# the3cloud/zktls

Hardware: AMD Instinct MI355X
Metric: trace-cells/s (higher is better)
Workload: dtype u32

## Files before the change

### zktls_amd/csrc/kernels.h

```cpp
#pragma once
#include <hip/hip_runtime.h>
#include <stddef.h>
#include <stdint.h>

#include "babybear.cuh"

namespace zk {

struct NttPassArgs {
    const uint32_t* in;
    uint32_t* out;
    uint64_t in_ld, out_ld;
    uint32_t ncols;
    uint32_t num_tiles;
    uint32_t log_m;
    uint64_t in_tile_mul, in_stride;
    uint64_t out_tile_mul, out_stride;
    uint32_t bitrev_out;
    uint32_t map_mode;
    uint64_t tile_perm;
    uint32_t fast_path;
    uint32_t debug_flags;
    uint32_t cols_per_thread;
    uint32_t bench_tag;
// ... 169 lines not shown
    uint32_t inv_zh[4];
    const uint32_t* body;
    uint32_t n_constraints;
    const uint32_t* weights;
    const uint32_t* pub;
    uint32_t* out;
    uint32_t* lde_out; uint64_t lde_ld;
    const uint32_t* recs; uint32_t n_terms; uint32_t n_public;
    const uint32_t* addend;
    uint32_t no_chain;
    uint32_t wide;
    uint32_t cls[6];
};
constexpr uint32_t AIR_WIDE_POINTS = 64, AIR_WIDE_PITCH = 65;
inline bool air_wide_form(uint32_t width, uint32_t n_terms, int log_n, uint32_t n_public) {
    return n_terms >= 2048 && width % 4 == 0 && (size_t)AIR_WIDE_PITCH * (width + AIR_SLOT_EXTRA + n_public) * 4 <= 160 * 1024 && log_n >= 6;
}
ZK_HD uint32_t air_wide_word(uint32_t slot, uint32_t W) {
    if (slot < W) return AIR_WIDE_PITCH * slot;
    if (slot < 2 * W) return AIR_WIDE_PITCH * (slot - W) + 1u;
    return AIR_WIDE_PITCH * (W + (slot - 2 * W));
}
hipError_t launch_quotient_air(const QuotientAirArgs& a, hipStream_t s);

hipError_t launch_inv_denominators(const uint32_t* xs, uint64_t count, const Ext& z0, const Ext& z1, int npoints,
                                   uint32_t* out, uint32_t* xw, uint64_t xw_count, hipStream_t s);

struct OpenArgs {
    const uint32_t* mat;
    uint64_t ld;
    uint32_t width;
    uint64_t rows;
    const uint32_t* xw;
    uint64_t xw_stride;
    uint32_t* partial;
    int tx;
};
size_t open_chunks(uint64_t rows, uint32_t width, uint64_t ld, const uint32_t* mat);
hipError_t launch_open(const OpenArgs& a, int npts, const Ext& scale0, const Ext& scale1, uint32_t* out, hipStream_t s);

struct ReducedArgs {
    const uint32_t* tlde; uint64_t t_ld; uint32_t width;
    const uint32_t* qlde; uint64_t q_ld; uint32_t q_width;
    const uint32_t* plde; uint64_t p_ld; uint32_t p_width;
    uint64_t rows;
    const uint32_t* alpha_pow;
    const uint32_t* dinv;
    Ext y_loc, y_next, y_pl, y_pn, y_q, off_next, off_pl, off_pn, off_q;
    Ext off_loc;
    int accumulate;
    uint32_t* out;
};
hipError_t launch_reduced_opening(const ReducedArgs& a, uint32_t* scratch_at, hipStream_t s);

struct PermArgs {
    const uint32_t* trace; uint64_t ld;
    uint64_t rows; uint32_t pairs;
    Ext gamma, beta;
    uint32_t* out; uint64_t out_ld;
};
hipError_t launch_perm_trace(const PermArgs& a, uint32_t* block_scratch, hipStream_t s);

constexpr int LOOKUP_REC_WORDS = 12;
struct LookupArgs {
    const uint32_t* table; uint32_t ni, cols;
    Ext gamma, bpow[9];
    const uint8_t* cmap; uint32_t n_used, chunk_mask;
};
constexpr uint32_t LOOKUP_MAX_COLS = 512, LOOKUP_STAGE_MAX_USED = 56;
struct MachinePermArgs {
    LookupArgs lk;
    const uint32_t* trace; uint64_t ld; uint64_t rows;
    uint32_t* out; uint64_t out_ld;
    const uint32_t* pre; uint64_t pre_ld; uint32_t pre_w;
};
bool lookup_perm_two_sources_ok(const MachinePermArgs& a);
hipError_t launch_perm_trace_machine(const MachinePermArgs& a, uint32_t* block_scratch, hipStream_t s);
struct MachineQuotArgs {
    LookupArgs lk;
    const uint32_t* lde; uint64_t ld; const uint32_t* perm; uint64_t perm_ld; int log_n;
    int log_qd;
    const uint32_t* xs; const uint32_t* sel_first; const uint32_t* sel_last; uint32_t wn_inv;
    const uint32_t* weights;
    Ext cumsum;
    uint32_t* addend;
};
hipError_t launch_lookup_addend(const MachineQuotArgs& a, hipStream_t s);

hipError_t launch_fri_fold(const uint32_t* in, uint32_t* out, const uint32_t* itw, uint64_t half, const Ext& beta, hipStream_t s);
hipError_t launch_ext_add(uint32_t* dst, const uint32_t* src, uint64_t count, hipStream_t s);
hipError_t launch_fri_fold_dev(const uint32_t* in, uint32_t* out, const uint32_t* itw, uint64_t half, const uint32_t* beta_ptr,
                               int squarings, hipStream_t s);

struct DevChallenger {
    uint32_t state[16];
    uint32_t in[8];
    uint32_t out[8];
    int32_t n_in, n_out;
};
hipError_t launch_fri_challenge(DevChallenger* chal, const uint32_t* root, uint32_t* beta_out, uint32_t* root_log, hipStream_t s);


struct GrindArgs {
    uint32_t state[16];
    int slot;
    uint32_t mask;
// ... 15 lines not shown
```

### zktls_amd/csrc/prover.cpp

```cpp
#include <atomic>
#include <chrono>
#include <condition_variable>
#include <deque>
#include <cstring>
#include <functional>
#include <mutex>
#include <string>
#include <thread>
#include <vector>

#include "proof_common.h"
#include "batch.h"

namespace zk { std::atomic<bool> g_fri_graph{true}; }
namespace zk {

extern std::atomic<uint64_t> g_p2_generation;
void air_digest_cached(const AirView& a, uint32_t out[8]) {
    struct Entry { std::vector<uint32_t> words; uint64_t generation; uint32_t dg[8]; };
    static std::mutex mu;
    static std::vector<Entry> cache;
    const uint64_t gen = g_p2_generation.load();
    {
        std::lock_guard<std::mutex> lk(mu);
// ... 429 lines not shown
int zkhip_fri_fold_k(zkhip_ctx* ctx, const uint32_t* d_in, int log_h, int log_arity, const uint32_t beta[4], uint32_t* d_out) {
    CHECK_CTX(ctx);
    if (!d_in || !d_out || !beta || log_arity < 1 || log_arity > 6 || log_h < log_arity || log_h > MAX_LOG_ROWS + 3)
        return fail(ZKHIP_ERR_INVALID, "fri_fold_k: bad arguments");
    ZK_TRY(ensure_fold_table(ctx, log_h));
    void* tmp;
    ZK_TRY(ctx_reserve(ctx, S_PARTIAL, ((size_t)1 << log_h) * 16, &tmp));
    uint32_t* ping = (uint32_t*)tmp;
    uint32_t* pong = ping + ((size_t)2 << log_h);
    Ext b{{beta[0], beta[1], beta[2], beta[3]}};
    const uint32_t* src = d_in;
    for (int j = 0; j < log_arity; j++) {
        const int lh = log_h - j;
        uint32_t* dst = (j == log_arity - 1) ? d_out : ((j & 1) ? pong : ping);
        ZK_HIP(launch_fri_fold(src, dst, ctx->dom_itw, (uint64_t)1 << (lh - 1), b, ctx->stream));
        src = dst;
        b = ext_mul(b, b);
    }
    return ZKHIP_OK;
}

int zkhip_request_digest(const uint8_t* input, size_t input_len, const uint8_t* program, size_t program_len, uint32_t out[8]) {
    if (!out || (input_len && !input) || (program_len && !program)) return fail(ZKHIP_ERR_INVALID, "request_digest: null pointer");
    uint32_t st[16] = {0};
    int pos = 0;
    auto absorb = [&](uint32_t canonical) {
        st[pos++] = to_monty(canonical);
        if (pos == 8) { p2_permute(st); pos = 0; }
    };
    auto absorb_bytes = [&](const uint8_t* b, size_t n) {
        absorb((uint32_t)(n & 0xFFFFFF));
        absorb((uint32_t)((uint64_t)n >> 24) & 0xFFFFFF);
        for (size_t i = 0; i < n; i += 3) {
            uint32_t v = b[i];
            if (i + 1 < n) v |= (uint32_t)b[i + 1] << 8;
            if (i + 2 < n) v |= (uint32_t)b[i + 2] << 16;
            absorb(v);
        }
    };
    absorb(0x5A4B54);
    absorb_bytes(input, input_len);
    absorb_bytes(program, program_len);
    if (pos) p2_permute(st);
    for (int i = 0; i < 8; i++) out[i] = from_monty(st[i]);
    return ZKHIP_OK;
}

size_t zkhip_proof_size(int log_n, uint32_t width, const zkhip_params* prm, size_t n_public) {
    (void)n_public;
    if (check_shape(log_n, width, prm) != ZKHIP_OK) return 0;
    return proof_words(log_n, width, prm) * 4;
}

static int prove_shard_impl(zkhip_ctx* ctx, const uint32_t* d_trace, size_t ld, int log_n, uint32_t width,
                            const uint32_t* public_values, size_t n_public, const zkhip_params* prm,
                            uint8_t* proof, size_t cap, size_t* len, const AirView* air) {
    CHECK_CTX(ctx);
    ZK_TRY(check_shape(log_n, width, prm));
    if (!d_trace || !proof || !len || ld < width || (n_public && !public_values)) return fail(ZKHIP_ERR_INVALID, "prove_shard: bad arguments");
    for (size_t i = 0; i < n_public; i++) if (public_values[i] >= P) return fail(ZKHIP_ERR_INVALID, "prove_shard: public values must be canonical");
    if (air && prm->logup_pairs) return fail(ZKHIP_ERR_INVALID, "prove_shard_air: a constraint program excludes the built-in lookup argument (logup_pairs must be 0)");
    if (air && prm->code_width) return fail(ZKHIP_ERR_INVALID, "prove_shard_air: the code / data group split belongs to the built-in prover (code_width must be 0)");
    const int lqd = air ? air->lqd : 1;
    if (lqd > prm->log_blowup) return fail(ZKHIP_ERR_INVALID, "prove_shard_air: constraints of degree 4 or 5 need log_blowup >= 2 (the quotient domain must lie inside the committed LDE domain)");
    const size_t NQ = (size_t)1 << lqd, QW = 4 * NQ;
    const size_t need = proof_words(log_n, width, prm, air != nullptr, lqd) * 4;
    if (cap < need) return fail(ZKHIP_ERR_BUFFER, "prove_shard: proof buffer too small (see zkhip_proof_size)");
    *len = 0;
    Shape sh;
    shape_of(log_n, prm, sh);
    const int H = log_n + sh.b, Hq = log_n + lqd, Q = prm->num_queries;
    const int RL = sh.R, K = sh.K;
    const size_t n = (size_t)1 << log_n, m = (size_t)1 << H, arity = (size_t)1 << K;
    hipStream_t st = ctx->stream;
    ZK_TRY(ensure_domain(ctx, log_n, sh.b));

    uint32_t* pf = (uint32_t*)proof;
    size_t pos = 0;
    const uint32_t LQ = (uint32_t)prm->logup_pairs;
    const size_t wp = LQ ? 4 * ((size_t)LQ + 1) : 0;
    const uint32_t CW = sh.cw;
    pf[pos++] = PROOF_MAGIC; pf[pos++] = air ? 7u : (CW ? 8u : (sh.ext ? 3u : (LQ ? 2u : PROOF_VERSION))); pf[pos++] = (uint32_t)log_n; pf[pos++] = width;
    pf[pos++] = (uint32_t)prm->log_blowup; pf[pos++] = (uint32_t)Q; pf[pos++] = (uint32_t)prm->pow_bits; pf[pos++] = (uint32_t)n_public;
    if (sh.ext || air) { pf[pos++] = LQ; pf[pos++] = (uint32_t)sh.K; pf[pos++] = (uint32_t)sh.F; pf[pos++] = (uint32_t)sh.hw; }
    else if (LQ) pf[pos++] = LQ;
    if (air) { air_digest_cached(*air, pf + pos); pos += 8; }
    if (CW) pf[pos++] = CW;

    Challenger ch;
    transcript_init(ch, log_n, width, prm, n_public, sh, air);
    uint32_t root[8];

    void *v_tlde, *v_ttree;
    ZK_TRY(ctx_reserve(ctx, S_TLDE, m * width * 4, &v_tlde));
    ZK_TRY(ctx_reserve(ctx, S_TTREE, (2 * m - 1) * 32, &v_ttree));
    uint32_t* tlde = (uint32_t*)v_tlde; uint32_t* ttree = (uint32_t*)v_ttree;
    ZK_TRY(op_coset_lde(ctx, d_trace, ld, tlde, width, log_n, width, sh.b, MONTY_GEN));
    uint32_t* ctree = nullptr;
    if (CW) {
        void* v_ctree;
        ZK_TRY(ctx_reserve(ctx, S_CTREE, (2 * m - 1) * 32, &v_ctree));
        ctree = (uint32_t*)v_ctree;
        ZK_TRY(commit_hw(ctx, tlde, width, CW, H, ctree, sh.hw));
        ZK_TRY(d2h(ctx, root, ctree + (2 * m - 2) * 8, 32));
        for (int i = 0; i < 8; i++) { ch.observe(root[i]); pf[pos++] = from_monty(root[i]); }
        ZK_TRY(commit_hw(ctx, tlde + CW, width, width - CW, H, ttree, sh.hw));
// ... 53 lines not shown
    uint32_t* dinv = (uint32_t*)v_dinv; uint32_t* d_open = (uint32_t*)v_open;
    uint32_t* xw = dinv + 8 * m;
    ZK_HIP(launch_inv_denominators(ctx->dom_xs, m, zpts[0], zpts[1], 2, dinv, xw, n, st));
    ZK_TRY(run_open(ctx, tlde, width, log_n, width, zpts, 2, xw, d_open));
    ZK_TRY(dev_sync(ctx));
    if (LQ) {
        ZK_TRY(run_open(ctx, plde, wp, log_n, (uint32_t)wp, zpts, 2, xw, d_open + 8 * (size_t)width));
        ZK_TRY(dev_sync(ctx));
    }
    ZK_TRY(run_open(ctx, qlde, QW, log_n, (uint32_t)QW, zpts, 1, xw, d_open + 8 * (size_t)width + 8 * wp));
    std::vector<uint32_t> opened((2 * (size_t)width + 2 * wp + QW) * 4);
    ZK_TRY(d2h(ctx, opened.data(), d_open, opened.size() * 4));
    observe_words(ch, opened.data(), opened.size());
    for (size_t i = 0; i < opened.size(); i++) pf[pos++] = from_monty(opened[i]);
    const Ext* op_loc = (const Ext*)opened.data();
    const Ext* op_nxt = op_loc + width;
    const Ext* op_pl = op_nxt + width;
    const Ext* op_pn = op_pl + wp;
    const Ext* op_q = op_pn + wp;

    const Ext fa = ch.sample_ext();
    size_t np = width > QW ? width : QW;
    if (wp > np) np = wp;
    std::vector<Ext> fapow(np);
    fapow[0] = ext_one();
    for (size_t j = 1; j < np; j++) fapow[j] = ext_mul(fapow[j - 1], fa);
    ReducedArgs ra{};
    ra.y_loc = ra.y_next = ra.y_pl = ra.y_pn = ra.y_q = ext_zero();
    ra.off_loc = ext_one(); ra.accumulate = 0;
    for (size_t j = 0; j < width; j++) {
        ra.y_loc = ext_add(ra.y_loc, ext_mul(fapow[j], op_loc[j]));
        ra.y_next = ext_add(ra.y_next, ext_mul(fapow[j], op_nxt[j]));
    }
    for (size_t j = 0; j < wp; j++) {
        ra.y_pl = ext_add(ra.y_pl, ext_mul(fapow[j], op_pl[j]));
        ra.y_pn = ext_add(ra.y_pn, ext_mul(fapow[j], op_pn[j]));
    }
    for (size_t j = 0; j < QW; j++) ra.y_q = ext_add(ra.y_q, ext_mul(fapow[j], op_q[j]));
    ra.off_next = ext_pow(fa, width);
    ra.off_pl = ext_pow(fa, 2 * (uint64_t)width);
    ra.off_pn = ext_pow(fa, 2 * (uint64_t)width + wp);
    ra.off_q = ext_pow(fa, 2 * (uint64_t)width + 2 * wp);
    void *v_apf, *v_layers, *v_ltrees;
    ZK_TRY(ctx_reserve(ctx, S_APOW_F, np * 16, &v_apf));
    ZK_TRY(h2d(ctx, v_apf, fapow.data(), np * 16));
    ZK_TRY(ctx_reserve(ctx, S_FRI_LAYERS, 2 * m * 16, &v_layers));
    ZK_TRY(ctx_reserve(ctx, S_FRI_TREES, 2 * m * 32, &v_ltrees));
    uint32_t* layers = (uint32_t*)v_layers; uint32_t* ltrees = (uint32_t*)v_ltrees;
    ra.tlde = tlde; ra.t_ld = width; ra.width = width; ra.qlde = qlde; ra.q_ld = QW; ra.q_width = (uint32_t)QW; ra.rows = m;
    ra.plde = plde; ra.p_ld = wp; ra.p_width = (uint32_t)wp;
    ra.alpha_pow = (const uint32_t*)v_apf; ra.dinv = dinv; ra.out = layers;
    void* v_at;
    ZK_TRY(ctx_reserve(ctx, S_PARTIAL, 2 * m * 16, &v_at));
    ZK_HIP(launch_reduced_opening(ra, (uint32_t*)v_at, st));

    std::vector<size_t> layer_off(RL + 1), tree_off(RL + 1);
    {
        size_t lo = 0, to = 0;
        for (int l = 0; l <= RL; l++) {
            layer_off[l] = lo; tree_off[l] = to;
            lo += ((size_t)1 << (H - K * l)) * 4;
            if (l < RL) to += (2 * ((size_t)1 << (H - K * (l + 1))) - 1) * 8;
        }
    }
    ZK_TRY(fri_commit_phase(ctx, ch, sh, H, RL, layers, ltrees, layer_off, tree_off, (uint32_t*)v_at, m, nullptr, pf, pos));
    {
        const int lf = sh.F + sh.b;
        const size_t nf = (size_t)1 << lf, keep = (size_t)1 << sh.F;
        std::vector<Ext> last(nf), nat(nf);
        ZK_TRY(d2h(ctx, last.data(), layers + layer_off[RL], nf * 16));
        for (size_t i = 0; i < nf; i++) nat[i] = last[reverse_bits((uint32_t)i, lf)];
        host_intt_ext(nat, lf);
        for (size_t i = keep; i < nf; i++)
            if (!ext_eq(nat[i], ext_zero()))
                return fail(ZKHIP_ERR_INVALID, "prove_shard: final FRI layer is not low-degree (the trace violates the AIR)");
        for (size_t i = 0; i < keep; i++) {
            for (int e = 0; e < 4; e++) pf[pos++] = from_monty(nat[i].c[e]);
            ch.observe_ext(nat[i]);
        }
    }

    uint32_t witness = 0;
    ZK_TRY(grind_witness(ctx, ch, prm->pow_bits, &witness));
    pf[pos++] = ctx->debug.pow_witness = witness;

    {
        std::vector<GatherDesc> descs;
        descs.reserve((size_t)Q * (4 + 4 * H + (size_t)RL * (H + arity)));
        size_t qpos = 0;
        auto push = [&](const uint32_t* src, size_t nwords) { descs.push_back(GatherDesc{src, (uint32_t)qpos, (uint32_t)nwords}); qpos += nwords; };
        auto push_path = [&](const uint32_t* tree, size_t leaves, size_t index, int levels) {
            const uint32_t* lvl = tree; size_t cnt = leaves, idx = index;
            for (int k = 0; k < levels; k++) { push(lvl + 8 * (idx ^ 1), 8); lvl += 8 * cnt; cnt >>= 1; idx >>= 1; }
        };
        for (int q = 0; q < Q; q++) {
            const size_t index = ch.sample_bits(H);
            push(tlde + index * width, width);
            if (CW) push_path(ctree, m, index, H);
            push_path(ttree, m, index, H);
            if (LQ) { push(plde + index * wp, wp); push_path(ptree, m, index, H); }
            push(qlde + index * QW, QW);
            push_path(qtree, m, index, H);
            size_t idx = index;
            for (int l = 0; l < RL; l++) {
                const int lh = H - K * (l + 1);
                const size_t row = idx >> K, own = idx & (arity - 1);
                for (size_t j = 0; j < arity; j++)
                    if (j != own) push(layers + layer_off[l] + (row * arity + j) * 4, 4);
                push_path(ltrees + tree_off[l], (size_t)1 << lh, row, lh);
                idx = row;
            }
        }
        if (pos + qpos != need / 4) return fail(ZKHIP_ERR_INTERNAL, "prove_shard: proof layout mismatch");
        void *v_desc, *v_out;
        ZK_TRY(ctx_reserve(ctx, S_GATHER_DESC, descs.size() * sizeof(GatherDesc), &v_desc));
        ZK_TRY(ctx_reserve(ctx, S_GATHER_OUT, qpos * 4, &v_out));
        ZK_TRY(h2d(ctx, v_desc, descs.data(), descs.size() * sizeof(GatherDesc)));
        ZK_HIP(launch_gather((const GatherDesc*)v_desc, (uint32_t)descs.size(), (uint32_t*)v_out, st));
        ZK_TRY(d2h(ctx, pf + pos, v_out, qpos * 4));
        pos += qpos;
    }
    for (int i = 0; i < 4; i++) {
        ctx->debug.alpha[i] = from_monty(alpha.c[i]);
        ctx->debug.zeta[i] = from_monty(zeta.c[i]);
        ctx->debug.fri_alpha[i] = from_monty(fa.c[i]);
    }
    *len = pos * 4;
    return ZKHIP_OK;
}

int zkhip_prove_shard(zkhip_ctx* ctx, const uint32_t* d_trace, size_t ld, int log_n, uint32_t width,
                      const uint32_t* public_values, size_t n_public, const zkhip_params* prm,
                      uint8_t* proof, size_t cap, size_t* len) {
    return prove_shard_impl(ctx, d_trace, ld, log_n, width, public_values, n_public, prm, proof, cap, len, nullptr);
}

size_t zkhip_proof_size_air(const uint32_t* program, size_t program_words, int log_n, uint32_t width, const zkhip_params* prm, size_t n_public) {
    AirView a;
    if (check_shape(log_n, width, prm) != ZKHIP_OK || prm->logup_pairs || !air_validate(program, program_words, width, n_public, &a) || a.lqd > prm->log_blowup) return 0;
    return proof_words(log_n, width, prm, true, a.lqd) * 4;
}
int zkhip_air_validate(const uint32_t* program, size_t words, uint32_t width, size_t n_public) {
    if (!air_validate(program, words, width, n_public, nullptr))
        return fail(ZKHIP_ERR_INVALID, "air_validate: malformed constraint program (header, selector, degree > 3, or a variable out of range)");
    return ZKHIP_OK;
}
int zkhip_air_digest(const uint32_t* program, size_t words, uint32_t out[8]) {
    AirView a;
    if (!out || !program || words < 6 || !air_validate(program, words, program[2], program[4], &a)) return fail(ZKHIP_ERR_INVALID, "air_digest: malformed constraint program");
    air_digest(a, out);
    return ZKHIP_OK;
}
int zkhip_air_synthetic(uint32_t width, size_t n_public, uint32_t* out, size_t cap, size_t* words) {
    if (!words || width == 0 || width % 4 != 0 || width > 1024) return fail(ZKHIP_ERR_INVALID, "air_synthetic: width must be a positive multiple of 4, at most 1024");
    const size_t G = width / 4, need = 6 + G * 33;
    *words = need;
    if (!out) return ZKHIP_OK;
    if (cap < need) return fail(ZKHIP_ERR_BUFFER, "air_synthetic: buffer too small");
    size_t p = 0;
    out[p++] = AIR_MAGIC; out[p++] = 1; out[p++] = width; out[p++] = (uint32_t)(3 * G); out[p++] = (uint32_t)n_public; out[p++] = (uint32_t)need;
    for (uint32_t g = 0; g < G; g++) {
        const uint32_t a = 4 * g, b = a + 1, c = a + 2, d = a + 3, NEXT = 1u << 30;
        out[p++] = 0; out[p++] = 3;
        out[p++] = 1; out[p++] = 1; out[p++] = c;
        out[p++] = P - 1; out[p++] = 3; out[p++] = a; out[p++] = a; out[p++] = b;
        out[p++] = P - (g + 1); out[p++] = 0;
        out[p++] = 3; out[p++] = 4;
        out[p++] = 1; out[p++] = 1; out[p++] = NEXT | d;
        out[p++] = P - 1; out[p++] = 2; out[p++] = a; out[p++] = b;
        out[p++] = P - 1; out[p++] = 1; out[p++] = c;
        out[p++] = P - (2 * g + 3); out[p++] = 0;
        out[p++] = 1; out[p++] = 2;
        out[p++] = 1; out[p++] = 1; out[p++] = d;
        out[p++] = P - (5 * g + 7); out[p++] = 0;
    }
    return p == need ? ZKHIP_OK : fail(ZKHIP_ERR_INTERNAL, "air_synthetic: layout mismatch");
}
int zkhip_prove_shard_air(zkhip_ctx* ctx, const uint32_t* program, size_t program_words, const uint32_t* d_trace, size_t ld, int log_n,
                          uint32_t width, const uint32_t* public_values, size_t n_public, const zkhip_params* prm,
                          uint8_t* proof, size_t cap, size_t* len) {
    AirView a;
    if (!air_validate(program, program_words, width, n_public, &a)) return fail(ZKHIP_ERR_INVALID, "prove_shard_air: malformed constraint program");
    return prove_shard_impl(ctx, d_trace, ld, log_n, width, public_values, n_public, prm, proof, cap, len, &a);
}
int zkhip_quotient_values_air(zkhip_ctx* ctx, const uint32_t* program, size_t program_words, const uint32_t* d_lde, size_t ld, int log_n,
                              uint32_t width, const uint32_t* public_values, size_t n_public, const uint32_t alpha[4], uint32_t* d_out) {
    CHECK_CTX(ctx);
    zkhip_params prm{1, 1, 0, 0, 0, 0, 0, 0};
// ... 622 lines not shown
```

### zktls_amd/csrc/stark.hip

```cpp
#include <atomic>

#include "poseidon2.cuh"
#include "kernels.h"
#include "batch.h"

namespace zk {

hipError_t stark_upload_p2_tables(const P2Tables& t, hipStream_t s) { return p2_upload_tables(t, s); }


ZK_D Ext ld_ext(const uint32_t* p) {
    uint4 v = *reinterpret_cast<const uint4*>(p);
    return Ext{{v.x, v.y, v.z, v.w}};
}
ZK_D void st_ext(uint32_t* p, const Ext& e) { *reinterpret_cast<uint4*>(p) = make_uint4(e.c[0], e.c[1], e.c[2], e.c[3]); }

ZK_D Ext group_sum(Ext v, int width) {
    for (int off = width >> 1; off > 0; off >>= 1) {
        Ext o;
        o.c[0] = __shfl_down(v.c[0], off, width);
        o.c[1] = __shfl_down(v.c[1], off, width);
        o.c[2] = __shfl_down(v.c[2], off, width);
        o.c[3] = __shfl_down(v.c[3], off, width);
        v = Ext{{dadd(v.c[0], o.c[0]), dadd(v.c[1], o.c[1]), dadd(v.c[2], o.c[2]), dadd(v.c[3], o.c[3])}};
// ... 847 lines not shown
            uint4* dst = reinterpret_cast<uint4*>(a.partial + 4 * (((uint64_t)blockIdx.x * NPTS + k) * a.width + col));
#pragma unroll
            for (int c = 0; c < 4; c++) dst[c] = make_uint4(mine[4 * c], mine[4 * c + 1], mine[4 * c + 2], mine[4 * c + 3]);
        }
    }
}
template <int NPTS>
__global__ void __launch_bounds__(256) open_partial4_kernel(OpenArgs a) { open_partial4_kernel_body<NPTS>(a); }
struct open_partial4_kernel_bargs { OpenArgs a; static open_partial4_kernel_bargs make(OpenArgs a) { return open_partial4_kernel_bargs{a}; } };
template <int NPTS>
__global__ void __launch_bounds__(256) open_partial4_kernel_batch(const open_partial4_kernel_bargs* __restrict__ zk_arr) { const open_partial4_kernel_bargs& zk_b = zk_arr[blockIdx.z]; open_partial4_kernel_body<NPTS>(zk_b.a); }

__device__ __forceinline__ void open_final_kernel_body(const uint32_t* partial, uint32_t nchunks, int npts, uint32_t width, const Ext& scale0, const Ext& scale1, uint32_t* out) {
    const uint32_t idx = blockIdx.x;
    const uint32_t k = idx / width, col = idx % width;
    Ext sum = ext_zero();
    for (uint32_t c = threadIdx.x; c < nchunks; c += 64) sum = ext_add(sum, ld_ext(partial + 4 * (((uint64_t)c * npts + k) * width + col)));
    sum = group_sum(sum, 64);
    if (threadIdx.x == 0) st_ext(out + 4 * (uint64_t)idx, ext_neg(ext_mul_dev(sum, k ? scale1 : scale0)));
}
__global__ void __launch_bounds__(64) open_final_kernel(const uint32_t* partial, uint32_t nchunks, int npts, uint32_t width, Ext scale0, Ext scale1, uint32_t* out) { open_final_kernel_body(partial, nchunks, npts, width, scale0, scale1, out); }
struct open_final_kernel_bargs { const uint32_t* partial; uint32_t nchunks; int npts; uint32_t width; Ext scale0; Ext scale1; uint32_t* out; static open_final_kernel_bargs make(const uint32_t* partial, uint32_t nchunks, int npts, uint32_t width, Ext scale0, Ext scale1, uint32_t* out) { return open_final_kernel_bargs{partial, nchunks, npts, width, scale0, scale1, out}; } };
__global__ void __launch_bounds__(64) open_final_kernel_batch(const open_final_kernel_bargs* __restrict__ zk_arr) { const open_final_kernel_bargs& zk_b = zk_arr[blockIdx.z]; open_final_kernel_body(zk_b.partial, zk_b.nchunks, zk_b.npts, zk_b.width, zk_b.scale0, zk_b.scale1, zk_b.out); }

bool open_uses_quads(uint32_t width, uint64_t ld, const uint32_t* mat) {
    return width >= 64 && width % 4 == 0 && ld % 4 == 0 && ((uintptr_t)mat & 15u) == 0;
}
size_t open_chunks(uint64_t rows, uint32_t width, uint64_t ld, const uint32_t* mat) {
    const uint64_t per = open_uses_quads(width, ld, mat) ? OPEN_ROWS4 : OPEN_ROWS;
    return (size_t)((rows + per - 1) / per);
}
hipError_t launch_open(const OpenArgs& a0, int npts, const Ext& scale0, const Ext& scale1, uint32_t* out, hipStream_t s) {
    OpenArgs a = a0;
    const bool quads = open_uses_quads(a.width, a.ld, a.mat);
    const uint32_t nchunks = (uint32_t)open_chunks(a.rows, a.width, a.ld, a.mat);
    if (quads) {
        a.tx = 1;
        while (a.tx < (int)(a.width / 4) && a.tx < 64) a.tx <<= 1;
        dim3 grid(nchunks, (a.width / 4 + a.tx - 1) / a.tx);
        if (npts == 1) ZK_LAUNCH(open_partial4_kernel<1>, open_partial4_kernel_batch<1>, open_partial4_kernel_bargs, grid, dim3(256), 0, s, a);
        else ZK_LAUNCH(open_partial4_kernel<2>, open_partial4_kernel_batch<2>, open_partial4_kernel_bargs, grid, dim3(256), 0, s, a);
    } else {
        dim3 grid(nchunks, (a.width + a.tx - 1) / a.tx);
        if (npts == 1) ZK_LAUNCH(open_partial_kernel<1>, open_partial_kernel_batch<1>, open_partial_kernel_bargs, grid, dim3(256), 0, s, a);
        else ZK_LAUNCH(open_partial_kernel<2>, open_partial_kernel_batch<2>, open_partial_kernel_bargs, grid, dim3(256), 0, s, a);
    }
    hipError_t e = hipGetLastError();
    if (e != hipSuccess) return e;
    const uint32_t n = (uint32_t)npts * a.width;
    ZK_LAUNCH(open_final_kernel, open_final_kernel_batch, open_final_kernel_bargs, dim3(n), dim3(64), 0, s, a.partial, nchunks, npts, a.width, scale0, scale1, out);
    return hipGetLastError();
}

__device__ __forceinline__ void rowdot_kernel_body(const uint32_t* __restrict__ mat, uint64_t ld, uint32_t width, uint64_t rows, int L, const uint32_t* __restrict__ alpha_pow, uint32_t* __restrict__ out_at) {
    const uint64_t gid = (uint64_t)blockIdx.x * blockDim.x + threadIdx.x;
    const uint64_t p = gid / L;
    const int lane = (int)(gid % L);
    if (p >= rows) return;
    const uint32_t* row = mat + p * ld;
    uint64_t acc[4] = {0, 0, 0, 0};
    const uint32_t nq = width / 4;
    for (uint32_t q = lane; q < nq; q += L) {
        const uint4 v = ld_stream(row + 4 * q);
        const uint4* ap = reinterpret_cast<const uint4*>(alpha_pow + 16 * q);
        const uint4 a0 = ap[0], a1 = ap[1], a2 = ap[2], a3 = ap[3];
        dacc2(acc[0], a0.x, v.x, a1.x, v.y); dacc2(acc[0], a2.x, v.z, a3.x, v.w);
        dacc2(acc[1], a0.y, v.x, a1.y, v.y); dacc2(acc[1], a2.y, v.z, a3.y, v.w);
        dacc2(acc[2], a0.z, v.x, a1.z, v.y); dacc2(acc[2], a2.z, v.z, a3.z, v.w);
        dacc2(acc[3], a0.w, v.x, a1.w, v.y); dacc2(acc[3], a2.w, v.z, a3.w, v.w);
    }
    Ext r;
#pragma unroll
    for (int i = 0; i < 4; i++) r.c[i] = row_group_sum(dacc_finish(acc[i]), L);
    if (lane == 0) st_ext(out_at + 4 * p, r);
}
__global__ void __launch_bounds__(256) rowdot_kernel(const uint32_t* __restrict__ mat, uint64_t ld, uint32_t width, uint64_t rows, int L, const uint32_t* __restrict__ alpha_pow, uint32_t* __restrict__ out_at) { rowdot_kernel_body(mat, ld, width, rows, L, alpha_pow, out_at); }
struct rowdot_kernel_bargs { const uint32_t* mat; uint64_t ld; uint32_t width; uint64_t rows; int L; const uint32_t* alpha_pow; uint32_t* out_at; static rowdot_kernel_bargs make(const uint32_t* mat, uint64_t ld, uint32_t width, uint64_t rows, int L, const uint32_t* alpha_pow, uint32_t* out_at) { return rowdot_kernel_bargs{mat, ld, width, rows, L, alpha_pow, out_at}; } };
__global__ void __launch_bounds__(256) rowdot_kernel_batch(const rowdot_kernel_bargs* __restrict__ zk_arr) { const rowdot_kernel_bargs& zk_b = zk_arr[blockIdx.z]; rowdot_kernel_body(zk_b.mat, zk_b.ld, zk_b.width, zk_b.rows, zk_b.L, zk_b.alpha_pow, zk_b.out_at); }

constexpr int ROWDOT_TRIPS = 16;
template <int NK>
__device__ __forceinline__ void rowdot_regs_kernel_body(const uint32_t* __restrict__ mat, uint64_t ld, uint32_t width, uint64_t rows, int L, const uint32_t* __restrict__ alpha_pow, uint32_t* __restrict__ out_at) {
    const int lane = (int)(threadIdx.x % L);
    const uint32_t nq = width / 4;
    const uint64_t rows_per_trip = 256 / L;
    const uint64_t r0 = (uint64_t)blockIdx.x * rows_per_trip * ROWDOT_TRIPS + threadIdx.x / L;
    uint4 a0[NK], a1[NK], a2[NK], a3[NK];
#pragma unroll
    for (int k = 0; k < NK; k++) {
        const uint32_t q = lane + (uint32_t)L * k;
        const uint4* ap = reinterpret_cast<const uint4*>(alpha_pow + 16 * (q < nq ? q : 0));
        a0[k] = ap[0]; a1[k] = ap[1]; a2[k] = ap[2]; a3[k] = ap[3];
    }
    for (int t = 0; t < ROWDOT_TRIPS; t++) {
        const uint64_t p = r0 + (uint64_t)t * rows_per_trip;
        if (p >= rows) return;
        const uint32_t* row = mat + p * ld;
        uint4 v[NK];
#pragma unroll
        for (int k = 0; k < NK; k++) {
            const uint32_t q = lane + (uint32_t)L * k;
            v[k] = q < nq ? ld_stream(row + 4 * q) : make_uint4(0, 0, 0, 0);
        }
        uint64_t acc[4] = {0, 0, 0, 0};
#pragma unroll
        for (int k = 0; k < NK; k++) {
            dacc2(acc[0], a0[k].x, v[k].x, a1[k].x, v[k].y); dacc2(acc[0], a2[k].x, v[k].z, a3[k].x, v[k].w);
            dacc2(acc[1], a0[k].y, v[k].x, a1[k].y, v[k].y); dacc2(acc[1], a2[k].y, v[k].z, a3[k].y, v[k].w);
            dacc2(acc[2], a0[k].z, v[k].x, a1[k].z, v[k].y); dacc2(acc[2], a2[k].z, v[k].z, a3[k].z, v[k].w);
            dacc2(acc[3], a0[k].w, v[k].x, a1[k].w, v[k].y); dacc2(acc[3], a2[k].w, v[k].z, a3[k].w, v[k].w);
        }
        Ext r;
#pragma unroll
        for (int i = 0; i < 4; i++) r.c[i] = row_group_sum(dacc_finish(acc[i]), L);
        if (lane == 0) st_ext(out_at + 4 * p, r);
    }
}
template <int NK>
__global__ void __launch_bounds__(256) rowdot_regs_kernel(const uint32_t* __restrict__ mat, uint64_t ld, uint32_t width, uint64_t rows, int L, const uint32_t* __restrict__ alpha_pow, uint32_t* __restrict__ out_at) { rowdot_regs_kernel_body<NK>(mat, ld, width, rows, L, alpha_pow, out_at); }
struct rowdot_regs_kernel_bargs { const uint32_t* mat; uint64_t ld; uint32_t width; uint64_t rows; int L; const uint32_t* alpha_pow; uint32_t* out_at; static rowdot_regs_kernel_bargs make(const uint32_t* mat, uint64_t ld, uint32_t width, uint64_t rows, int L, const uint32_t* alpha_pow, uint32_t* out_at) { return rowdot_regs_kernel_bargs{mat, ld, width, rows, L, alpha_pow, out_at}; } };
template <int NK>
__global__ void __launch_bounds__(256) rowdot_regs_kernel_batch(const rowdot_regs_kernel_bargs* __restrict__ zk_arr) { const rowdot_regs_kernel_bargs& zk_b = zk_arr[blockIdx.z]; rowdot_regs_kernel_body<NK>(zk_b.mat, zk_b.ld, zk_b.width, zk_b.rows, zk_b.L, zk_b.alpha_pow, zk_b.out_at); }

static hipError_t launch_rowdot(const uint32_t* mat, uint64_t ld, uint32_t width, uint64_t rows, const uint32_t* alpha_pow, uint32_t* out_at, hipStream_t s);
__device__ __forceinline__ void reduced_combine_kernel_body(const ReducedArgs& a, const uint32_t* __restrict__ at_in, const uint32_t* __restrict__ ap_in) {
    const uint64_t p = (uint64_t)blockIdx.x * blockDim.x + threadIdx.x;
    if (p >= a.rows) return;
    const Ext at = ld_ext(at_in + 4 * p);
    const uint4* qrow = reinterpret_cast<const uint4*>(a.qlde + p * a.q_ld);
    Ext aq = ext_zero();
    for (uint32_t h = 0; h < a.q_width / 8; h++) {
        const uint4 q0 = qrow[2 * h], q1 = qrow[2 * h + 1];
        const uint32_t qv[8] = {q0.x, q0.y, q0.z, q0.w, q1.x, q1.y, q1.z, q1.w};
#pragma unroll
        for (int j = 0; j < 8; j++) aq = ext_add(aq, ext_mul_base_dev(ld_ext(a.alpha_pow + 4 * (8 * h + j)), qv[j]));
    }
    const Ext d1 = ld_ext(a.dinv + 4 * p), d2 = ld_ext(a.dinv + 4 * (a.rows + p));
    Ext r = ext_mul_dev(a.off_loc, ext_mul_dev(ext_sub(at, a.y_loc), d1));
    r = ext_add(r, ext_mul_dev(a.off_next, ext_mul_dev(ext_sub(at, a.y_next), d2)));
    if (a.p_width) {
        const Ext ap = ld_ext(ap_in + 4 * p);
        r = ext_add(r, ext_mul_dev(a.off_pl, ext_mul_dev(ext_sub(ap, a.y_pl), d1)));
        r = ext_add(r, ext_mul_dev(a.off_pn, ext_mul_dev(ext_sub(ap, a.y_pn), d2)));
    }
    r = ext_add(r, ext_mul_dev(a.off_q, ext_mul_dev(ext_sub(aq, a.y_q), d1)));
    if (a.accumulate) r = ext_add(r, ld_ext(a.out + 4 * p));
    st_ext(a.out + 4 * p, r);
}
__global__ void __launch_bounds__(256) reduced_combine_kernel(ReducedArgs a, const uint32_t* __restrict__ at_in, const uint32_t* __restrict__ ap_in) { reduced_combine_kernel_body(a, at_in, ap_in); }
struct reduced_combine_kernel_bargs { ReducedArgs a; const uint32_t* at_in; const uint32_t* ap_in; static reduced_combine_kernel_bargs make(ReducedArgs a, const uint32_t* at_in, const uint32_t* ap_in) { return reduced_combine_kernel_bargs{a, at_in, ap_in}; } };
__global__ void __launch_bounds__(256) reduced_combine_kernel_batch(const reduced_combine_kernel_bargs* __restrict__ zk_arr) { const reduced_combine_kernel_bargs& zk_b = zk_arr[blockIdx.z]; reduced_combine_kernel_body(zk_b.a, zk_b.at_in, zk_b.ap_in); }

static int lanes_for(uint32_t width) { int g = (int)(width / 4), l = 1; while (l < g && l < 16) l <<= 1; return l; }
static hipError_t launch_rowdot(const uint32_t* mat, uint64_t ld, uint32_t width, uint64_t rows, const uint32_t* alpha_pow, uint32_t* out_at, hipStream_t s) {
    const int L = lanes_for(width);
    const uint32_t nq = width / 4;
    const int nk = (int)((nq + L - 1) / L);
    const uint64_t rows_per_wg = (uint64_t)(256 / L) * ROWDOT_TRIPS;
    if (nk <= 4 && rows % (256 / L) == 0 && rows >= rows_per_wg) {
        const dim3 grid((unsigned)((rows + rows_per_wg - 1) / rows_per_wg)), block(256);
        switch (nk) {
            case 1: ZK_LAUNCH(rowdot_regs_kernel<1>, rowdot_regs_kernel_batch<1>, rowdot_regs_kernel_bargs, grid, block, 0, s, mat, ld, width, rows, L, alpha_pow, out_at); break;
            case 2: ZK_LAUNCH(rowdot_regs_kernel<2>, rowdot_regs_kernel_batch<2>, rowdot_regs_kernel_bargs, grid, block, 0, s, mat, ld, width, rows, L, alpha_pow, out_at); break;
            case 3: ZK_LAUNCH(rowdot_regs_kernel<3>, rowdot_regs_kernel_batch<3>, rowdot_regs_kernel_bargs, grid, block, 0, s, mat, ld, width, rows, L, alpha_pow, out_at); break;
            default: ZK_LAUNCH(rowdot_regs_kernel<4>, rowdot_regs_kernel_batch<4>, rowdot_regs_kernel_bargs, grid, block, 0, s, mat, ld, width, rows, L, alpha_pow, out_at); break;
        }
        return hipGetLastError();
    }
    const uint64_t threads = rows * L;
    ZK_LAUNCH(rowdot_kernel, rowdot_kernel_batch, rowdot_kernel_bargs, dim3((unsigned)((threads + 255) / 256)), dim3(256), 0, s, mat, ld, width, rows, L, alpha_pow, out_at);
    return hipGetLastError();
}
hipError_t launch_reduced_opening(const ReducedArgs& a, uint32_t* scratch_at, hipStream_t s) {
    hipError_t e = launch_rowdot(a.tlde, a.t_ld, a.width, a.rows, a.alpha_pow, scratch_at, s);
    if (e != hipSuccess) return e;
    uint32_t* scratch_ap = scratch_at + 4 * a.rows;
    if (a.p_width) {
        e = launch_rowdot(a.plde, a.p_ld, a.p_width, a.rows, a.alpha_pow, scratch_ap, s);
        if (e != hipSuccess) return e;
    }
    ZK_LAUNCH(reduced_combine_kernel, reduced_combine_kernel_batch, reduced_combine_kernel_bargs, dim3((unsigned)((a.rows + 255) / 256)), dim3(256), 0, s, a, scratch_at, scratch_ap);
    return hipGetLastError();
}

constexpr int PERM_BLOCK = 256;
__device__ __forceinline__ void perm_rows_kernel_body(const PermArgs& a, uint32_t* __restrict__ block_tot) {
    __shared__ uint32_t sh[PERM_BLOCK * 4];
    const uint64_t i = (uint64_t)blockIdx.x * PERM_BLOCK + threadIdx.x;
    Ext sum = ext_zero();
    if (i < a.rows) {
        const uint32_t* row = a.trace + i * a.ld;
        uint32_t* prow = a.out + i * a.out_ld;
        for (uint32_t q = 0; q < a.pairs; q++) {
            const uint4 vs = *reinterpret_cast<const uint4*>(row + 8 * q);
            const uint4 vr = *reinterpret_cast<const uint4*>(row + 8 * q + 4);
            const Ext ds = ext_add(ext_add_base(a.gamma, vs.x), ext_mul_base_dev(a.beta, vs.y));
            const Ext dr = ext_add(ext_add_base(a.gamma, vr.x), ext_mul_base_dev(a.beta, vr.y));
            const Ext d = ext_mul_dev(ds, dr);
            const Ext phi = ext_eq(d, ext_zero()) ? ext_sub(ext_inv_dev(ds), ext_inv_dev(dr)) : ext_mul_dev(ext_sub(dr, ds), ext_inv_dev(d));
            st_ext(prow + 4 * q, phi);
            sum = ext_add(sum, phi);
        }
    }
    for (int k = 0; k < 4; k++) sh[threadIdx.x * 4 + k] = sum.c[k];
    __syncthreads();
    for (int off = 1; off < PERM_BLOCK; off <<= 1) {
        Ext o = ext_zero();
        if ((int)threadIdx.x >= off) o = Ext{{sh[(threadIdx.x - off) * 4], sh[(threadIdx.x - off) * 4 + 1], sh[(threadIdx.x - off) * 4 + 2], sh[(threadIdx.x - off) * 4 + 3]}};
        __syncthreads();
        sum = ext_add(sum, o);
        for (int k = 0; k < 4; k++) sh[threadIdx.x * 4 + k] = sum.c[k];
        __syncthreads();
    }
    if (i < a.rows) st_ext(a.out + i * a.out_ld + 4 * a.pairs, sum);
    if (threadIdx.x == PERM_BLOCK - 1) st_ext(block_tot + 4 * (uint64_t)blockIdx.x, sum);
}
__global__ void __launch_bounds__(PERM_BLOCK) perm_rows_kernel(PermArgs a, uint32_t* __restrict__ block_tot) { perm_rows_kernel_body(a, block_tot); }
struct perm_rows_kernel_bargs { PermArgs a; uint32_t* block_tot; static perm_rows_kernel_bargs make(PermArgs a, uint32_t* block_tot) { return perm_rows_kernel_bargs{a, block_tot}; } };
__global__ void __launch_bounds__(PERM_BLOCK) perm_rows_kernel_batch(const perm_rows_kernel_bargs* __restrict__ zk_arr) { const perm_rows_kernel_bargs& zk_b = zk_arr[blockIdx.z]; perm_rows_kernel_body(zk_b.a, zk_b.block_tot); }

__device__ __forceinline__ void perm_scan_blocks_kernel_body(uint32_t* block_tot, uint32_t nblocks) {
    __shared__ uint32_t sh[1024 * 4];
    const uint32_t per = (nblocks + 1023) / 1024;
    const uint32_t b0 = threadIdx.x * per;
    Ext sum = ext_zero();
    for (uint32_t k = 0; k < per && b0 + k < nblocks; k++) sum = ext_add(sum, ld_ext(block_tot + 4 * (uint64_t)(b0 + k)));
    for (int k = 0; k < 4; k++) sh[threadIdx.x * 4 + k] = sum.c[k];
    __syncthreads();
    Ext incl = sum;
    for (int off = 1; off < 1024; off <<= 1) {
        Ext o = ext_zero();
        if ((int)threadIdx.x >= off) o = Ext{{sh[(threadIdx.x - off) * 4], sh[(threadIdx.x - off) * 4 + 1], sh[(threadIdx.x - off) * 4 + 2], sh[(threadIdx.x - off) * 4 + 3]}};
        __syncthreads();
        incl = ext_add(incl, o);
// ... 289 lines not shown
```

Before: 20.20 billion.

## Compute reduced-opening row sums on one coset and extend the rest by LDE

With blowup 2 and a large trace, the row-dot over the full LDE matrix is replaced by a row-dot over the first half of the rows only. The row-dot kernel also writes those sums in natural order, and a coset LDE of that 4-column vector produces the second half. Because the row sum is linear in the columns, extending the sums gives the same result as summing the extended columns. This halves reads of the wide trace LDE for this stage, at the cost of a small extra 4-column NTT and a bit-reversed scatter store.

```diff
diff --git a/zktls_amd/csrc/kernels.h b/zktls_amd/csrc/kernels.h
--- a/zktls_amd/csrc/kernels.h
+++ b/zktls_amd/csrc/kernels.h
@@ -245,6 +245,8 @@
     uint32_t* out;
 };
 hipError_t launch_reduced_opening(const ReducedArgs& a, uint32_t* scratch_at, hipStream_t s);
+hipError_t launch_reduced_rowsums(const ReducedArgs& a, int log_rows, uint32_t* scratch_at, uint32_t* nat, hipStream_t s);
+hipError_t launch_reduced_combine(const ReducedArgs& a, const uint32_t* scratch_at, hipStream_t s);
 
 struct PermArgs {
     const uint32_t* trace; uint64_t ld;
diff --git a/zktls_amd/csrc/prover.cpp b/zktls_amd/csrc/prover.cpp
--- a/zktls_amd/csrc/prover.cpp
+++ b/zktls_amd/csrc/prover.cpp
@@ -505,6 +505,11 @@
     return proof_words(log_n, width, prm) * 4;
 }
 
+constexpr int REDUCED_COSET_MIN_LOG = 18;
+constexpr size_t REDUCED_COSET_MIN_CELLS = (size_t)1 << 26;
+#ifdef ZKHIP_AB_HOOKS
+static std::atomic<uint64_t> g_ab_reduced_coset_calls{0};
+#endif
 static int prove_shard_impl(zkhip_ctx* ctx, const uint32_t* d_trace, size_t ld, int log_n, uint32_t width,
                             const uint32_t* public_values, size_t n_public, const zkhip_params* prm,
                             uint8_t* proof, size_t cap, size_t* len, const AirView* air) {
@@ -664,7 +669,21 @@
     ra.alpha_pow = (const uint32_t*)v_apf; ra.dinv = dinv; ra.out = layers;
     void* v_at;
     ZK_TRY(ctx_reserve(ctx, S_PARTIAL, 2 * m * 16, &v_at));
-    ZK_HIP(launch_reduced_opening(ra, (uint32_t*)v_at, st));
+    bool rowsums_one_coset = sh.b == 1 && !LQ && log_n >= REDUCED_COSET_MIN_LOG && n * (size_t)width >= REDUCED_COSET_MIN_CELLS;
+#ifdef ZKHIP_AB_HOOKS
+    if (getenv("ZKHIP_REDUCED_FULL")) rowsums_one_coset = false;
+#endif
+    if (rowsums_one_coset) {
+#ifdef ZKHIP_AB_HOOKS
+        g_ab_reduced_coset_calls++;
+#endif
+        uint32_t* at = (uint32_t*)v_at;
+        ZK_HIP(launch_reduced_rowsums(ra, log_n, at, qchunk, st));
+        ZK_TRY(op_coset_lde(ctx, qchunk, 4, at + n * 4, 4, log_n, 4, 0, two_adic_generator(log_n + 1)));
+        ZK_HIP(launch_reduced_combine(ra, at, st));
+    } else {
+        ZK_HIP(launch_reduced_opening(ra, (uint32_t*)v_at, st));
+    }
 
     std::vector<size_t> layer_off(RL + 1), tree_off(RL + 1);
     {
@@ -746,6 +765,15 @@
                       uint8_t* proof, size_t cap, size_t* len) {
     return prove_shard_impl(ctx, d_trace, ld, log_n, width, public_values, n_public, prm, proof, cap, len, nullptr);
 }
+#ifdef ZKHIP_AB_HOOKS
+int zkhip_ab_fri_layer0(zkhip_ctx* ctx, uint32_t* out, size_t words) {
+    CHECK_CTX(ctx);
+    const DeviceBuffer& b = ctx->scratch[S_FRI_LAYERS];
+    if (!out || !b.ptr || b.bytes < words * 4) return fail(ZKHIP_ERR_INVALID, "ab_fri_layer0: no layer workspace of that size");
+    return d2h(ctx, out, b.ptr, words * 4);
+}
+uint64_t zkhip_ab_reduced_coset_calls(void) { return g_ab_reduced_coset_calls.load(); }
+#endif
 
 size_t zkhip_proof_size_air(const uint32_t* program, size_t program_words, int log_n, uint32_t width, const zkhip_params* prm, size_t n_public) {
     AirView a;
diff --git a/zktls_amd/csrc/stark.hip b/zktls_amd/csrc/stark.hip
--- a/zktls_amd/csrc/stark.hip
+++ b/zktls_amd/csrc/stark.hip
@@ -923,7 +923,7 @@
     return hipGetLastError();
 }
 
-__device__ __forceinline__ void rowdot_kernel_body(const uint32_t* __restrict__ mat, uint64_t ld, uint32_t width, uint64_t rows, int L, const uint32_t* __restrict__ alpha_pow, uint32_t* __restrict__ out_at) {
+__device__ __forceinline__ void rowdot_kernel_body(const uint32_t* __restrict__ mat, uint64_t ld, uint32_t width, uint64_t rows, int L, const uint32_t* __restrict__ alpha_pow, uint32_t* __restrict__ out_at, uint32_t* __restrict__ out_nat, int log_nat) {
     const uint64_t gid = (uint64_t)blockIdx.x * blockDim.x + threadIdx.x;
     const uint64_t p = gid / L;
     const int lane = (int)(gid % L);
@@ -943,15 +943,15 @@
     Ext r;
 #pragma unroll
     for (int i = 0; i < 4; i++) r.c[i] = row_group_sum(dacc_finish(acc[i]), L);
-    if (lane == 0) st_ext(out_at + 4 * p, r);
-}
-__global__ void __launch_bounds__(256) rowdot_kernel(const uint32_t* __restrict__ mat, uint64_t ld, uint32_t width, uint64_t rows, int L, const uint32_t* __restrict__ alpha_pow, uint32_t* __restrict__ out_at) { rowdot_kernel_body(mat, ld, width, rows, L, alpha_pow, out_at); }
-struct rowdot_kernel_bargs { const uint32_t* mat; uint64_t ld; uint32_t width; uint64_t rows; int L; const uint32_t* alpha_pow; uint32_t* out_at; static rowdot_kernel_bargs make(const uint32_t* mat, uint64_t ld, uint32_t width, uint64_t rows, int L, const uint32_t* alpha_pow, uint32_t* out_at) { return rowdot_kernel_bargs{mat, ld, width, rows, L, alpha_pow, out_at}; } };
-__global__ void __launch_bounds__(256) rowdot_kernel_batch(const rowdot_kernel_bargs* __restrict__ zk_arr) { const rowdot_kernel_bargs& zk_b = zk_arr[blockIdx.z]; rowdot_kernel_body(zk_b.mat, zk_b.ld, zk_b.width, zk_b.rows, zk_b.L, zk_b.alpha_pow, zk_b.out_at); }
+    if (lane == 0) { st_ext(out_at + 4 * p, r); if (out_nat) st_ext(out_nat + 4 * (uint64_t)(__brev((uint32_t)p) >> (32 - log_nat)), r); }
+}
+__global__ void __launch_bounds__(256) rowdot_kernel(const uint32_t* __restrict__ mat, uint64_t ld, uint32_t width, uint64_t rows, int L, const uint32_t* __restrict__ alpha_pow, uint32_t* __restrict__ out_at, uint32_t* __restrict__ out_nat, int log_nat) { rowdot_kernel_body(mat, ld, width, rows, L, alpha_pow, out_at, out_nat, log_nat); }
+struct rowdot_kernel_bargs { const uint32_t* mat; uint64_t ld; uint32_t width; uint64_t rows; int L; const uint32_t* alpha_pow; uint32_t* out_at; uint32_t* out_nat; int log_nat; static rowdot_kernel_bargs make(const uint32_t* mat, uint64_t ld, uint32_t width, uint64_t rows, int L, const uint32_t* alpha_pow, uint32_t* out_at, uint32_t* out_nat, int log_nat) { return rowdot_kernel_bargs{mat, ld, width, rows, L, alpha_pow, out_at, out_nat, log_nat}; } };
+__global__ void __launch_bounds__(256) rowdot_kernel_batch(const rowdot_kernel_bargs* __restrict__ zk_arr) { const rowdot_kernel_bargs& zk_b = zk_arr[blockIdx.z]; rowdot_kernel_body(zk_b.mat, zk_b.ld, zk_b.width, zk_b.rows, zk_b.L, zk_b.alpha_pow, zk_b.out_at, zk_b.out_nat, zk_b.log_nat); }
 
 constexpr int ROWDOT_TRIPS = 16;
 template <int NK>
-__device__ __forceinline__ void rowdot_regs_kernel_body(const uint32_t* __restrict__ mat, uint64_t ld, uint32_t width, uint64_t rows, int L, const uint32_t* __restrict__ alpha_pow, uint32_t* __restrict__ out_at) {
+__device__ __forceinline__ void rowdot_regs_kernel_body(const uint32_t* __restrict__ mat, uint64_t ld, uint32_t width, uint64_t rows, int L, const uint32_t* __restrict__ alpha_pow, uint32_t* __restrict__ out_at, uint32_t* __restrict__ out_nat, int log_nat) {
     const int lane = (int)(threadIdx.x % L);
     const uint32_t nq = width / 4;
     const uint64_t rows_per_trip = 256 / L;
@@ -984,16 +984,15 @@
         Ext r;
 #pragma unroll
         for (int i = 0; i < 4; i++) r.c[i] = row_group_sum(dacc_finish(acc[i]), L);
-        if (lane == 0) st_ext(out_at + 4 * p, r);
+        if (lane == 0) { st_ext(out_at + 4 * p, r); if (out_nat) st_ext(out_nat + 4 * (uint64_t)(__brev((uint32_t)p) >> (32 - log_nat)), r); }
     }
 }
 template <int NK>
-__global__ void __launch_bounds__(256) rowdot_regs_kernel(const uint32_t* __restrict__ mat, uint64_t ld, uint32_t width, uint64_t rows, int L, const uint32_t* __restrict__ alpha_pow, uint32_t* __restrict__ out_at) { rowdot_regs_kernel_body<NK>(mat, ld, width, rows, L, alpha_pow, out_at); }
-struct rowdot_regs_kernel_bargs { const uint32_t* mat; uint64_t ld; uint32_t width; uint64_t rows; int L; const uint32_t* alpha_pow; uint32_t* out_at; static rowdot_regs_kernel_bargs make(const uint32_t* mat, uint64_t ld, uint32_t width, uint64_t rows, int L, const uint32_t* alpha_pow, uint32_t* out_at) { return rowdot_regs_kernel_bargs{mat, ld, width, rows, L, alpha_pow, out_at}; } };
+__global__ void __launch_bounds__(256) rowdot_regs_kernel(const uint32_t* __restrict__ mat, uint64_t ld, uint32_t width, uint64_t rows, int L, const uint32_t* __restrict__ alpha_pow, uint32_t* __restrict__ out_at, uint32_t* __restrict__ out_nat, int log_nat) { rowdot_regs_kernel_body<NK>(mat, ld, width, rows, L, alpha_pow, out_at, out_nat, log_nat); }
+struct rowdot_regs_kernel_bargs { const uint32_t* mat; uint64_t ld; uint32_t width; uint64_t rows; int L; const uint32_t* alpha_pow; uint32_t* out_at; uint32_t* out_nat; int log_nat; static rowdot_regs_kernel_bargs make(const uint32_t* mat, uint64_t ld, uint32_t width, uint64_t rows, int L, const uint32_t* alpha_pow, uint32_t* out_at, uint32_t* out_nat, int log_nat) { return rowdot_regs_kernel_bargs{mat, ld, width, rows, L, alpha_pow, out_at, out_nat, log_nat}; } };
 template <int NK>
-__global__ void __launch_bounds__(256) rowdot_regs_kernel_batch(const rowdot_regs_kernel_bargs* __restrict__ zk_arr) { const rowdot_regs_kernel_bargs& zk_b = zk_arr[blockIdx.z]; rowdot_regs_kernel_body<NK>(zk_b.mat, zk_b.ld, zk_b.width, zk_b.rows, zk_b.L, zk_b.alpha_pow, zk_b.out_at); }
-
-static hipError_t launch_rowdot(const uint32_t* mat, uint64_t ld, uint32_t width, uint64_t rows, const uint32_t* alpha_pow, uint32_t* out_at, hipStream_t s);
+__global__ void __launch_bounds__(256) rowdot_regs_kernel_batch(const rowdot_regs_kernel_bargs* __restrict__ zk_arr) { const rowdot_regs_kernel_bargs& zk_b = zk_arr[blockIdx.z]; rowdot_regs_kernel_body<NK>(zk_b.mat, zk_b.ld, zk_b.width, zk_b.rows, zk_b.L, zk_b.alpha_pow, zk_b.out_at, zk_b.out_nat, zk_b.log_nat); }
+
 __device__ __forceinline__ void reduced_combine_kernel_body(const ReducedArgs& a, const uint32_t* __restrict__ at_in, const uint32_t* __restrict__ ap_in) {
     const uint64_t p = (uint64_t)blockIdx.x * blockDim.x + threadIdx.x;
     if (p >= a.rows) return;
@@ -1023,7 +1022,7 @@
 __global__ void __launch_bounds__(256) reduced_combine_kernel_batch(const reduced_combine_kernel_bargs* __restrict__ zk_arr) { const reduced_combine_kernel_bargs& zk_b = zk_arr[blockIdx.z]; reduced_combine_kernel_body(zk_b.a, zk_b.at_in, zk_b.ap_in); }
 
 static int lanes_for(uint32_t width) { int g = (int)(width / 4), l = 1; while (l < g && l < 16) l <<= 1; return l; }
-static hipError_t launch_rowdot(const uint32_t* mat, uint64_t ld, uint32_t width, uint64_t rows, const uint32_t* alpha_pow, uint32_t* out_at, hipStream_t s) {
+static hipError_t launch_rowdot(const uint32_t* mat, uint64_t ld, uint32_t width, uint64_t rows, const uint32_t* alpha_pow, uint32_t* out_at, uint32_t* out_nat, int log_nat, hipStream_t s) {
     const int L = lanes_for(width);
     const uint32_t nq = width / 4;
     const int nk = (int)((nq + L - 1) / L);
@@ -1031,26 +1030,34 @@
     if (nk <= 4 && rows % (256 / L) == 0 && rows >= rows_per_wg) {
         const dim3 grid((unsigned)((rows + rows_per_wg - 1) / rows_per_wg)), block(256);
         switch (nk) {
-            case 1: ZK_LAUNCH(rowdot_regs_kernel<1>, rowdot_regs_kernel_batch<1>, rowdot_regs_kernel_bargs, grid, block, 0, s, mat, ld, width, rows, L, alpha_pow, out_at); break;
-            case 2: ZK_LAUNCH(rowdot_regs_kernel<2>, rowdot_regs_kernel_batch<2>, rowdot_regs_kernel_bargs, grid, block, 0, s, mat, ld, width, rows, L, alpha_pow, out_at); break;
-            case 3: ZK_LAUNCH(rowdot_regs_kernel<3>, rowdot_regs_kernel_batch<3>, rowdot_regs_kernel_bargs, grid, block, 0, s, mat, ld, width, rows, L, alpha_pow, out_at); break;
-            default: ZK_LAUNCH(rowdot_regs_kernel<4>, rowdot_regs_kernel_batch<4>, rowdot_regs_kernel_bargs, grid, block, 0, s, mat, ld, width, rows, L, alpha_pow, out_at); break;
+            case 1: ZK_LAUNCH(rowdot_regs_kernel<1>, rowdot_regs_kernel_batch<1>, rowdot_regs_kernel_bargs, grid, block, 0, s, mat, ld, width, rows, L, alpha_pow, out_at, out_nat, log_nat); break;
+            case 2: ZK_LAUNCH(rowdot_regs_kernel<2>, rowdot_regs_kernel_batch<2>, rowdot_regs_kernel_bargs, grid, block, 0, s, mat, ld, width, rows, L, alpha_pow, out_at, out_nat, log_nat); break;
+            case 3: ZK_LAUNCH(rowdot_regs_kernel<3>, rowdot_regs_kernel_batch<3>, rowdot_regs_kernel_bargs, grid, block, 0, s, mat, ld, width, rows, L, alpha_pow, out_at, out_nat, log_nat); break;
+            default: ZK_LAUNCH(rowdot_regs_kernel<4>, rowdot_regs_kernel_batch<4>, rowdot_regs_kernel_bargs, grid, block, 0, s, mat, ld, width, rows, L, alpha_pow, out_at, out_nat, log_nat); break;
         }
         return hipGetLastError();
     }
     const uint64_t threads = rows * L;
-    ZK_LAUNCH(rowdot_kernel, rowdot_kernel_batch, rowdot_kernel_bargs, dim3((unsigned)((threads + 255) / 256)), dim3(256), 0, s, mat, ld, width, rows, L, alpha_pow, out_at);
+    ZK_LAUNCH(rowdot_kernel, rowdot_kernel_batch, rowdot_kernel_bargs, dim3((unsigned)((threads + 255) / 256)), dim3(256), 0, s, mat, ld, width, rows, L, alpha_pow, out_at, out_nat, log_nat);
     return hipGetLastError();
 }
 hipError_t launch_reduced_opening(const ReducedArgs& a, uint32_t* scratch_at, hipStream_t s) {
-    hipError_t e = launch_rowdot(a.tlde, a.t_ld, a.width, a.rows, a.alpha_pow, scratch_at, s);
+    hipError_t e = launch_rowdot(a.tlde, a.t_ld, a.width, a.rows, a.alpha_pow, scratch_at, nullptr, 0, s);
     if (e != hipSuccess) return e;
     uint32_t* scratch_ap = scratch_at + 4 * a.rows;
     if (a.p_width) {
-        e = launch_rowdot(a.plde, a.p_ld, a.p_width, a.rows, a.alpha_pow, scratch_ap, s);
+        e = launch_rowdot(a.plde, a.p_ld, a.p_width, a.rows, a.alpha_pow, scratch_ap, nullptr, 0, s);
         if (e != hipSuccess) return e;
     }
     ZK_LAUNCH(reduced_combine_kernel, reduced_combine_kernel_batch, reduced_combine_kernel_bargs, dim3((unsigned)((a.rows + 255) / 256)), dim3(256), 0, s, a, scratch_at, scratch_ap);
+    return hipGetLastError();
+}
+hipError_t launch_reduced_rowsums(const ReducedArgs& a, int log_rows, uint32_t* scratch_at, uint32_t* nat, hipStream_t s) {
+    if (a.p_width || log_rows < 1 || log_rows > 31 || ((uint64_t)1 << log_rows) > a.rows) return hipErrorInvalidValue;
+    return launch_rowdot(a.tlde, a.t_ld, a.width, (uint64_t)1 << log_rows, a.alpha_pow, scratch_at, nat, log_rows, s);
+}
+hipError_t launch_reduced_combine(const ReducedArgs& a, const uint32_t* scratch_at, hipStream_t s) {
+    ZK_LAUNCH(reduced_combine_kernel, reduced_combine_kernel_batch, reduced_combine_kernel_bargs, dim3((unsigned)((a.rows + 255) / 256)), dim3(256), 0, s, a, scratch_at, scratch_at + 4 * a.rows);
     return hipGetLastError();
 }
 
```

After: 20.49 billion, median of 6. 1.01x the previous value.
